# apcamargo/genomad

Measured on NVIDIA H100. Metric: nn_classification_windows_per_s, higher is better.
Workload: dtype split operands on wgmma (conv: fp16 main pass + two e4m3 correction passes; w_v: 3 fp16 passes), fp32 accumulate; fp32-equivalent (<=1e-4 vs the fp32 oracle, measured ~1e-5)

## Files before the change

### genomad_b200/csrc/common.cuh

```cuda
#pragma once
#include <cuda_runtime.h>
#include <cuda_fp16.h>
#include <cuda_fp8.h>
#include <stdint.h>
#include "wgmma.cuh"

namespace gnm {

constexpr int kWindow   = 6000;
constexpr int kTok      = 5997;
constexpr int kVocab    = 257;
constexpr int kC        = 128;
constexpr int kTaps     = 6;
constexpr int kPatches  = 2100;
constexpr int kPatchLen = 4;
constexpr int kPool     = 8;
constexpr int kPooled   = 749;
constexpr int kHidden   = 512;
constexpr float kLeaky  = 0.1f;

constexpr int kRowBytes  = 768;
constexpr int kOffHi16   = 0, kOffLo16 = 256, kOffP8 = 512;
constexpr float kActScale = 32.f;
constexpr float kLo8Scale = 128.f;
constexpr float kHi8Scale = 4.f;
constexpr float kHi8Limit = 448.f / kHi8Scale;
constexpr float kF16Limit = 65504.f;

__device__ __forceinline__ uint32_t smem_u32(const void* p) {
  return static_cast<uint32_t>(__cvta_generic_to_shared(p));
}
__device__ __forceinline__ float lrelu(float x) { return x > 0.f ? x : x * kLeaky; }

__device__ __forceinline__ void split_f16(float x, __half& hi, __half& lo) {
  hi = __float2half_rn(x);
  lo = __float2half_rn(x - __half2float(hi));
}
__device__ __forceinline__ uint32_t pack_h2(__half a, __half b) {
  return static_cast<uint32_t>(__half_as_ushort(a)) | (static_cast<uint32_t>(__half_as_ushort(b)) << 16);
}

__device__ __forceinline__ void split2_f16(float a, float b, __half2& hi, __half2& lo) {
  hi = __floats2half2_rn(a, b);
  const float2 f = __half22float2(hi);
  lo = __floats2half2_rn(a - f.x, b - f.y);
}

__device__ __forceinline__ uint16_t pack_e4m3x2(float a, float b) {
  return static_cast<uint16_t>(__nv_cvt_float2_to_fp8x2(make_float2(a, b), __NV_SATFINITE, __NV_E4M3));
}

__device__ __forceinline__ void stmatrix_x4_trans(uint32_t saddr, uint32_t r0, uint32_t r1, uint32_t r2, uint32_t r3) {
  asm volatile("stmatrix.sync.aligned.m8n8.x4.trans.shared.b16 [%0], {%1, %2, %3, %4};"
               ::"r"(saddr), "r"(r0), "r"(r1), "r"(r2), "r"(r3) : "memory");
}
__device__ __forceinline__ uint4 ld_shared_v4(uint32_t saddr) {
  uint4 v;
  asm volatile("ld.shared.v4.b32 {%0, %1, %2, %3}, [%4];" : "=r"(v.x), "=r"(v.y), "=r"(v.z), "=r"(v.w) : "r"(saddr) : "memory");
  return v;
}

struct DeviceStatus { int code; int info0; int info1; int info2; int act_overflow; int ov_stage[4]; };
enum : int { kDevOk = 0, kDevMbarTimeout = 1 };
__device__ __forceinline__ void flag_act_overflow(DeviceStatus* st, float absmax, float limit, int stage) {
  if (absmax > limit && st) { st->act_overflow = 1; st->ov_stage[stage] = 1; }
}

__device__ __forceinline__ bool elect_one() {
  uint32_t pred;
  asm volatile(
      "{\n\t.reg .pred P;\n\t"
      "elect.sync _|P, 0xffffffff;\n\t"
      "selp.u32 %0, 1, 0, P;\n\t}"
      : "=r"(pred));
  return pred != 0;
}

__device__ __forceinline__ void mbar_init(uint64_t* bar, uint32_t count) {
  asm volatile("mbarrier.init.shared::cta.b64 [%0], %1;" ::"r"(smem_u32(bar)), "r"(count));
}
__device__ __forceinline__ void fence_barrier_init() {
  asm volatile("fence.mbarrier_init.release.cluster;" ::: "memory");
}
__device__ __forceinline__ void fence_proxy_async_smem() {
  asm volatile("fence.proxy.async.shared::cta;" ::: "memory");
}
__device__ __forceinline__ void mbar_arrive_expect_tx(uint64_t* bar, uint32_t bytes) {
  asm volatile("mbarrier.arrive.expect_tx.shared::cta.b64 _, [%0], %1;" ::"r"(smem_u32(bar)), "r"(bytes) : "memory");
}
__device__ __forceinline__ void mbar_arrive(uint64_t* bar) {
  asm volatile("mbarrier.arrive.shared::cta.b64 _, [%0];" ::"r"(smem_u32(bar)) : "memory");
}
__device__ __forceinline__ bool mbar_try_wait(uint64_t* bar, uint32_t parity) {
  uint32_t ok;
  asm volatile(
      "{\n\t.reg .pred p;\n\t"
      "mbarrier.try_wait.parity.shared::cta.b64 p, [%1], %2, %3;\n\t"
      "selp.u32 %0, 1, 0, p;\n\t}"
      : "=r"(ok) : "r"(smem_u32(bar)), "r"(parity), "r"(20000u) : "memory");
  return ok != 0;
}
__device__ __forceinline__ void mbar_wait(uint64_t* bar, uint32_t parity, DeviceStatus* st, int tag) {
  if (mbar_try_wait(bar, parity)) return;
  const long long t0 = clock64();
  for (uint32_t spins = 1;; ++spins) {
    if (mbar_try_wait(bar, parity)) return;
    if ((spins & 255u) == 0 && clock64() - t0 > 4000000000LL) {
      if (st) { st->code = kDevMbarTimeout; st->info0 = tag; st->info1 = blockIdx.x; st->info2 = threadIdx.x; }
      __threadfence_system();
      __trap();
    }
  }
}

__device__ __forceinline__ void tma_prefetch_desc(const void* tmap) {
  asm volatile("prefetch.tensormap [%0];" ::"l"(reinterpret_cast<uint64_t>(tmap)) : "memory");
}
__device__ __forceinline__ uint64_t l2_policy_evict_last() {
  uint64_t p;
  asm volatile("createpolicy.fractional.L2::evict_last.b64 %0, 1.0;" : "=l"(p));
  return p;
}
__device__ __forceinline__ uint64_t l2_policy_evict_first() {
  uint64_t p;
  asm volatile("createpolicy.fractional.L2::evict_first.b64 %0, 1.0;" : "=l"(p));
  return p;
}
__device__ __forceinline__ void tma_load_2d_hint(void* smem_dst, const void* tmap, uint64_t* bar, int c0, int c1, uint64_t policy) {
  asm volatile(
      "cp.async.bulk.tensor.2d.shared::cluster.global.mbarrier::complete_tx::bytes.L2::cache_hint [%0], [%1, {%3, %4}], [%2], %5;"
      ::"r"(smem_u32(smem_dst)), "l"(reinterpret_cast<uint64_t>(tmap)), "r"(smem_u32(bar)), "r"(c0), "r"(c1), "l"(policy)
      : "memory");
}
__device__ __forceinline__ void tma_load_3d_hint(void* smem_dst, const void* tmap, uint64_t* bar, int c0, int c1, int c2, uint64_t policy) {
  asm volatile(
      "cp.async.bulk.tensor.3d.shared::cluster.global.mbarrier::complete_tx::bytes.L2::cache_hint [%0], [%1, {%3, %4, %5}], [%2], %6;"
      ::"r"(smem_u32(smem_dst)), "l"(reinterpret_cast<uint64_t>(tmap)), "r"(smem_u32(bar)), "r"(c0), "r"(c1), "r"(c2), "l"(policy)
      : "memory");
}
}
```

### genomad_b200/csrc/wgmma.cuh

```cuda
#pragma once
#include <stdint.h>

namespace gnm {

__device__ __forceinline__ void wgmma_fence() { asm volatile("wgmma.fence.sync.aligned;" ::: "memory"); }
__device__ __forceinline__ void wgmma_commit() { asm volatile("wgmma.commit_group.sync.aligned;" ::: "memory"); }
template <int kPending> __device__ __forceinline__ void wgmma_wait() {
  asm volatile("wgmma.wait_group.sync.aligned %0;" ::"n"(kPending) : "memory");
}
template <int kN> __device__ __forceinline__ void wgmma_fence_regs(float (&d)[kN]) {
#pragma unroll
  for (int i = 0; i < kN; ++i) asm volatile("" : "+f"(d[i])::"memory");
}

__device__ __forceinline__ uint64_t gmma_desc_sw128(uint32_t saddr) {
  uint64_t d = 0;
  d |= static_cast<uint64_t>((saddr & 0x3FFFF) >> 4);
  d |= static_cast<uint64_t>(1) << 16;
  d |= static_cast<uint64_t>(1024 >> 4) << 32;
  d |= static_cast<uint64_t>(1) << 62;
  return d;
}

#define GNM_ACC8(b) "+f"(d[b]), "+f"(d[b + 1]), "+f"(d[b + 2]), "+f"(d[b + 3]), "+f"(d[b + 4]), "+f"(d[b + 5]), "+f"(d[b + 6]), "+f"(d[b + 7])
__device__ __forceinline__ void wgmma_f16_n48(float (&d)[24], uint64_t da, uint64_t db, uint32_t accumulate) {
  asm volatile("{\n.reg .pred p;\nsetp.ne.b32 p, %26, 0;\n"
               "wgmma.mma_async.sync.aligned.m64n48k16.f32.f16.f16 {%0,%1,%2,%3,%4,%5,%6,%7,%8,%9,%10,%11,%12,%13,%14,%15,%16,%17,%18,%19,%20,%21,%22,%23}, %24,%25,p,1,1,0,0;\n}"
               : GNM_ACC8(0), GNM_ACC8(8), GNM_ACC8(16)
               : "l"(da), "l"(db), "r"(accumulate));
}
__device__ __forceinline__ void wgmma_f16_n192(float (&d)[96], uint64_t da, uint64_t db, uint32_t accumulate) {
  asm volatile("{\n.reg .pred p;\nsetp.ne.b32 p, %98, 0;\n"
               "wgmma.mma_async.sync.aligned.m64n192k16.f32.f16.f16 {%0,%1,%2,%3,%4,%5,%6,%7,%8,%9,%10,%11,%12,%13,%14,%15,%16,%17,%18,%19,%20,%21,%22,%23,%24,%25,%26,%27,%28,%29,%30,%31,%32,%33,%34,%35,%36,%37,%38,%39,%40,%41,%42,%43,%44,%45,%46,%47,%48,%49,%50,%51,%52,%53,%54,%55,%56,%57,%58,%59,%60,%61,%62,%63,%64,%65,%66,%67,%68,%69,%70,%71,%72,%73,%74,%75,%76,%77,%78,%79,%80,%81,%82,%83,%84,%85,%86,%87,%88,%89,%90,%91,%92,%93,%94,%95}, %96,%97,p,1,1,0,0;\n}"
               : GNM_ACC8(0), GNM_ACC8(8), GNM_ACC8(16), GNM_ACC8(24), GNM_ACC8(32), GNM_ACC8(40), GNM_ACC8(48), GNM_ACC8(56), GNM_ACC8(64), GNM_ACC8(72), GNM_ACC8(80), GNM_ACC8(88)
               : "l"(da), "l"(db), "r"(accumulate));
}
__device__ __forceinline__ void wgmma_f16_n256(float (&d)[128], uint64_t da, uint64_t db, uint32_t accumulate) {
  asm volatile("{\n.reg .pred p;\nsetp.ne.b32 p, %130, 0;\n"
               "wgmma.mma_async.sync.aligned.m64n256k16.f32.f16.f16 {%0,%1,%2,%3,%4,%5,%6,%7,%8,%9,%10,%11,%12,%13,%14,%15,%16,%17,%18,%19,%20,%21,%22,%23,%24,%25,%26,%27,%28,%29,%30,%31,%32,%33,%34,%35,%36,%37,%38,%39,%40,%41,%42,%43,%44,%45,%46,%47,%48,%49,%50,%51,%52,%53,%54,%55,%56,%57,%58,%59,%60,%61,%62,%63,%64,%65,%66,%67,%68,%69,%70,%71,%72,%73,%74,%75,%76,%77,%78,%79,%80,%81,%82,%83,%84,%85,%86,%87,%88,%89,%90,%91,%92,%93,%94,%95,%96,%97,%98,%99,%100,%101,%102,%103,%104,%105,%106,%107,%108,%109,%110,%111,%112,%113,%114,%115,%116,%117,%118,%119,%120,%121,%122,%123,%124,%125,%126,%127}, %128,%129,p,1,1,0,0;\n}"
               : GNM_ACC8(0), GNM_ACC8(8), GNM_ACC8(16), GNM_ACC8(24), GNM_ACC8(32), GNM_ACC8(40), GNM_ACC8(48), GNM_ACC8(56), GNM_ACC8(64), GNM_ACC8(72), GNM_ACC8(80), GNM_ACC8(88), GNM_ACC8(96), GNM_ACC8(104), GNM_ACC8(112), GNM_ACC8(120)
               : "l"(da), "l"(db), "r"(accumulate));
}
__device__ __forceinline__ void wgmma_e4m3_n256(float (&d)[128], uint64_t da, uint64_t db, uint32_t accumulate) {
  asm volatile("{\n.reg .pred p;\nsetp.ne.b32 p, %130, 0;\n"
               "wgmma.mma_async.sync.aligned.m64n256k32.f32.e4m3.e4m3 {%0,%1,%2,%3,%4,%5,%6,%7,%8,%9,%10,%11,%12,%13,%14,%15,%16,%17,%18,%19,%20,%21,%22,%23,%24,%25,%26,%27,%28,%29,%30,%31,%32,%33,%34,%35,%36,%37,%38,%39,%40,%41,%42,%43,%44,%45,%46,%47,%48,%49,%50,%51,%52,%53,%54,%55,%56,%57,%58,%59,%60,%61,%62,%63,%64,%65,%66,%67,%68,%69,%70,%71,%72,%73,%74,%75,%76,%77,%78,%79,%80,%81,%82,%83,%84,%85,%86,%87,%88,%89,%90,%91,%92,%93,%94,%95,%96,%97,%98,%99,%100,%101,%102,%103,%104,%105,%106,%107,%108,%109,%110,%111,%112,%113,%114,%115,%116,%117,%118,%119,%120,%121,%122,%123,%124,%125,%126,%127}, %128,%129,p,1,1;\n}"
               : GNM_ACC8(0), GNM_ACC8(8), GNM_ACC8(16), GNM_ACC8(24), GNM_ACC8(32), GNM_ACC8(40), GNM_ACC8(48), GNM_ACC8(56), GNM_ACC8(64), GNM_ACC8(72), GNM_ACC8(80), GNM_ACC8(88), GNM_ACC8(96), GNM_ACC8(104), GNM_ACC8(112), GNM_ACC8(120)
               : "l"(da), "l"(db), "r"(accumulate));
}
__device__ __forceinline__ void wgmma_tf32_n256(float (&d)[128], uint64_t da, uint64_t db, uint32_t accumulate) {
  asm volatile("{\n.reg .pred p;\nsetp.ne.b32 p, %130, 0;\n"
               "wgmma.mma_async.sync.aligned.m64n256k8.f32.tf32.tf32 {%0,%1,%2,%3,%4,%5,%6,%7,%8,%9,%10,%11,%12,%13,%14,%15,%16,%17,%18,%19,%20,%21,%22,%23,%24,%25,%26,%27,%28,%29,%30,%31,%32,%33,%34,%35,%36,%37,%38,%39,%40,%41,%42,%43,%44,%45,%46,%47,%48,%49,%50,%51,%52,%53,%54,%55,%56,%57,%58,%59,%60,%61,%62,%63,%64,%65,%66,%67,%68,%69,%70,%71,%72,%73,%74,%75,%76,%77,%78,%79,%80,%81,%82,%83,%84,%85,%86,%87,%88,%89,%90,%91,%92,%93,%94,%95,%96,%97,%98,%99,%100,%101,%102,%103,%104,%105,%106,%107,%108,%109,%110,%111,%112,%113,%114,%115,%116,%117,%118,%119,%120,%121,%122,%123,%124,%125,%126,%127}, %128,%129,p,1,1;\n}"
               : GNM_ACC8(0), GNM_ACC8(8), GNM_ACC8(16), GNM_ACC8(24), GNM_ACC8(32), GNM_ACC8(40), GNM_ACC8(48), GNM_ACC8(56), GNM_ACC8(64), GNM_ACC8(72), GNM_ACC8(80), GNM_ACC8(88), GNM_ACC8(96), GNM_ACC8(104), GNM_ACC8(112), GNM_ACC8(120)
               : "l"(da), "l"(db), "r"(accumulate));
}
#undef GNM_ACC8

}
```

### genomad_b200/csrc/wv_gather.cuh

```cuda
#pragma once
#include <cuda.h>
#include <type_traits>
#include "common.cuh"
#include "conv_t.cuh"
#include "igloo.cuh"

namespace gnm {

constexpr int kBandRows   = 24;
constexpr int kBandWins   = 8;
constexpr int kWgN        = kBandRows * kBandWins;
constexpr int kNumBands   = (kTok + kBandRows - 1) / kBandRows;
constexpr int kWgRegion   = kWgN * 128;
constexpr int kWgBufs     = 6;
constexpr int kWgSlab     = kWgBufs * kWgRegion;
constexpr int kWgWBytes   = kWvStages * kBStage;
constexpr int kWgMmaWarps = 8;
constexpr int kWgWarps    = 7;
constexpr int kWgThreads  = (kWgMmaWarps + kWgWarps + 1) * 32;
constexpr int kWgGroupCap = 4;
constexpr int kWgGroupMax = 4;
constexpr int kWgSmem     = kWgSlab + kWgWBytes + 2048;
static_assert(kWgSmem <= 232448, "wv_gather_kernel exceeds the 227 KB of shared memory a CTA may use");
static_assert(kWgN == 3 * 64 && kBandRows == 3 * kPool && kBandWins == 8, "unit shape: three pool groups of 8 positions x 8 windows");
static_assert(kWgRegion % 1024 == 0, "regions must keep the 1024-byte alignment of the 128-byte swizzle");

struct WvGatherParams {
  float* q_out;
  float out_scale;
  const int2* grp;
  const int32_t* band_gstart;
  const uint4* wfrag;
  float gather_unscale;
  float* part_t;
  int n_windows, n_pad;
  int groups;
  int n_units;
  const int32_t* cta_split;
  int experiment;
  long long* dbg;
  DeviceStatus* status;
};

__device__ __forceinline__ uint2 ldg_frag(const uint2* p) {
  uint2 v;
  asm volatile("ld.global.nc.L1::evict_last.v2.u32 {%0, %1}, [%2];" : "=r"(v.x), "=r"(v.y) : "l"(p));
  return v;
}
__device__ __forceinline__ void ldsm_x4(uint32_t saddr, uint32_t (&a)[4]) {
  asm volatile("ldmatrix.sync.aligned.m8n8.x4.shared.b16 {%0, %1, %2, %3}, [%4];"
               : "=r"(a[0]), "=r"(a[1]), "=r"(a[2]), "=r"(a[3]) : "r"(saddr));
}
__device__ __forceinline__ void mma_16816(float (&d)[4], const uint32_t (&a)[4], uint32_t b0, uint32_t b1) {
  asm volatile("mma.sync.aligned.m16n8k16.row.col.f32.f16.f16.f32 {%0, %1, %2, %3}, {%4, %5, %6, %7}, {%8, %9}, {%0, %1, %2, %3};"
               : "+f"(d[0]), "+f"(d[1]), "+f"(d[2]), "+f"(d[3]) : "r"(a[0]), "r"(a[1]), "r"(a[2]), "r"(a[3]), "r"(b0), "r"(b1));
}

__global__ void __launch_bounds__(kWgThreads, 1)
wv_gather_kernel(const __grid_constant__ CUtensorMap tm_band, const __grid_constant__ CUtensorMap tm_w, const WvGatherParams p) {
  extern __shared__ uint8_t smem_raw[];
  uint8_t* smem = reinterpret_cast<uint8_t*>((reinterpret_cast<uintptr_t>(smem_raw) + 1023) & ~uintptr_t(1023));
  uint8_t* s_a = smem;
  uint8_t* s_w = smem + kWgSlab;
  uint64_t* bars = reinterpret_cast<uint64_t*>(s_w + kWgWBytes);
  uint64_t* a_full = bars;
  uint64_t* a_empty = bars + 8;
  uint64_t* w_full = bars + 16;

  const int warp = __shfl_sync(0xffffffffu, static_cast<int>(threadIdx.x) >> 5, 0);
  const int lane = threadIdx.x & 31;
  constexpr int kProducerWarp = kWgMmaWarps + kWgWarps;
  const int u_begin = p.cta_split[blockIdx.x], u_end = p.cta_split[blockIdx.x + 1];

  if (warp == kProducerWarp && elect_one()) {
    tma_prefetch_desc(&tm_band);
    tma_prefetch_desc(&tm_w);
    for (int i = 0; i < kWgBufs; ++i) { mbar_init(&a_full[i], 1); mbar_init(&a_empty[i], kWgMmaWarps + kWgWarps); }
    mbar_init(w_full, 1);
    fence_barrier_init();
  }
  __syncthreads();

  if (warp == kProducerWarp) {
    if (elect_one()) {
      mbar_arrive_expect_tx(w_full, kWgWBytes);
      for (int q = 0; q < kWvStages; ++q) tma_load_2d_hint(s_w + q * kBStage, &tm_w, w_full, 0, q * 128, l2_policy_evict_last());
      const uint64_t pol = l2_policy_evict_first();
      uint32_t phases = 0;
      int b0 = 0;
      long long c_wait_empty = 0;
      for (int unit = u_begin; unit < u_end; ++unit) {
        const int band = unit / p.groups;
        const int w0 = (unit - band * p.groups) * kBandWins;
#pragma unroll
        for (int k = 0; k < 4; ++k) {
          int b = b0 + k; if (b >= kWgBufs) b -= kWgBufs;
          const long long tq = clock64();
          mbar_wait(&a_empty[b], ((phases >> b) & 1) ^ 1, p.status, 500 + b);
          c_wait_empty += clock64() - tq;
          phases ^= 1u << b;
          mbar_arrive_expect_tx(&a_full[b], kWgRegion);
          const int src = (k & 1 ? kOffLo16 : kOffHi16) + (k >> 1) * 128;
          tma_load_3d_hint(s_a + b * kWgRegion, &tm_band, &a_full[b], src, w0, band * kBandRows, pol);
        }
        b0 += 4; if (b0 >= kWgBufs) b0 -= kWgBufs;
      }
      if (p.dbg) p.dbg[blockIdx.x * 8 + 7] = c_wait_empty;
    }
  } else if (warp < kWgMmaWarps) {
    const int g = warp >> 2, wq = warp & 3;
    const uint32_t a_base = smem_u32(s_a);
    const uint32_t w_base = smem_u32(s_w) + g * 64 * 128;
    const int ch0 = g * 64 + wq * 16 + (lane >> 2);
    const int win0 = 2 * (lane & 3);
    const float oscale = p.out_scale;
    mbar_wait(w_full, 0, p.status, 510);
    uint32_t phases = 0;
    int b0 = 0;
    uint32_t w_a = 0, t_mma = 0, t_epi = 0;
    float d[96];
    for (int unit = u_begin; unit < u_end; ++unit) {
      auto buf = [&](int k) { const int b = b0 + k; return b >= kWgBufs ? b - kWgBufs : b; };
      const uint32_t t_unit = clock();
#pragma unroll
      for (int kh = 0; kh < 2; ++kh) {
#pragma unroll
        for (int r = 0; r < 2; ++r) {
          const int b = buf(2 * kh + r);
          const uint32_t tq = clock();
          mbar_wait(&a_full[b], (phases >> b) & 1, p.status, 530 + b);
          w_a += clock() - tq;
          phases ^= 1u << b;
        }
        const uint64_t yh = gmma_desc_sw128(a_base + buf(2 * kh) * kWgRegion);
        const uint64_t yl = gmma_desc_sw128(a_base + buf(2 * kh + 1) * kWgRegion);
        const uint64_t whi = gmma_desc_sw128(w_base + (2 * kh) * kBStage);
        const uint64_t wlo = gmma_desc_sw128(w_base + (2 * kh + 1) * kBStage);
        wgmma_fence();
#pragma unroll
        for (int kk = 0; kk < 4; ++kk) {
          wgmma_f16_n192(d, whi + kk * 2, yh + kk * 2, (kh == 0 && kk == 0) ? 0u : 1u);
          wgmma_f16_n192(d, whi + kk * 2, yl + kk * 2, 1u);
        }
#pragma unroll
        for (int kk = 0; kk < 4; ++kk) wgmma_f16_n192(d, wlo + kk * 2, yh + kk * 2, 1u);
        wgmma_commit();
      }
      wgmma_wait<1>();
      __syncwarp();
      if (lane == 0) { mbar_arrive(&a_empty[buf(0)]); mbar_arrive(&a_empty[buf(1)]); }
      wgmma_wait<0>();
      wgmma_fence_regs(d);
      const uint32_t t_epi0 = clock();
      t_mma += t_epi0 - t_unit;
      const int band = unit / p.groups;
      const int w0 = (unit - band * p.groups) * kBandWins;
#pragma unroll
      for (int pg = 0; pg < kBandRows / kPool; ++pg) {
        const int gg = band * (kBandRows / kPool) + pg;
        if (gg < kPooled && !(p.experiment & 128)) {
#pragma unroll
          for (int h = 0; h < 2; ++h)
#pragma unroll
            for (int e = 0; e < 2; ++e) {
              float m = d[32 * pg + 2 * h + e];
#pragma unroll
              for (int i = 1; i < kPool; ++i) m = fmaxf(m, d[32 * pg + 4 * i + 2 * h + e]);
              const int w = w0 + win0 + e;
              if (w < p.n_windows) p.q_out[(static_cast<size_t>(w) * kPooled + gg) * kC + ch0 + 8 * h] = m * oscale;
            }
        }
      }
      __syncwarp();
      if (lane == 0) { mbar_arrive(&a_empty[buf(2)]); mbar_arrive(&a_empty[buf(3)]); }
      t_epi += clock() - t_epi0;
      b0 += 4; if (b0 >= kWgBufs) b0 -= kWgBufs;
    }
    if (p.dbg && warp == 0 && lane == 0) { long long* o = p.dbg + blockIdx.x * 8; o[3] = t_mma; o[4] = w_a; o[6] = t_epi; }
  } else {
    const int gw = warp - kWgMmaWarps;
    const float gscale = p.gather_unscale;
    const int lm_plane = (lane >> 3) & 1, lm_chunk = lane >> 4, lm_win = lane & 7;
    const int gid = lane >> 2, tig = lane & 3;
    const uint32_t slab = smem_u32(s_a);
    int it = 0;
    uint32_t phases = 0;
    int b0 = 0;
    long long c_wait_full = 0, c_gather = 0, tq = 0;
    const long long t_begin = clock64();
    int cur_band = -1, g_first = 0, g_cnt = 0, n_mine = 0;
    int my_e0[kWgGroupCap] = {}, my_meta[kWgGroupCap] = {};
    bool fast = true;
    struct GroupFrag { uint2 b[4]; uint32_t a[4][4]; };
    auto load_group = [&](int e0, int meta, int kh, uint32_t hi_base, uint32_t lo_base, GroupFrag& f) {
      const int row = meta & 31, ne = meta >> 8;
      const uint2* wf = reinterpret_cast<const uint2*>(p.wfrag) + ((static_cast<size_t>(e0 + (gid >> 1)) * 2 + kh) * 16 + tig) * 2 + (gid & 1);
#pragma unroll
      for (int ks = 0; ks < 4; ++ks) f.b[ks] = ((gid >> 1) < ne && !(p.experiment & 1024)) ? ldg_frag(wf + ks * 8) : make_uint2(0u, 0u);
      const uint32_t rb = (lm_plane ? lo_base : hi_base) + row * (kBandWins * 128) + lm_win * 128;
#pragma unroll
      for (int ks = 0; ks < 4; ++ks) {
        if (p.experiment & 2048) { f.a[ks][0] = f.a[ks][1] = f.a[ks][2] = f.a[ks][3] = rb; continue; }
        ldsm_x4(rb + (((ks * 2 + lm_chunk) ^ lm_win) << 4), f.a[ks]);
      }
    };
    auto mma_group = [&](const GroupFrag& f) -> float {
      float d[4][4];
#pragma unroll
      for (int ks = 0; ks < 4; ++ks) d[ks][0] = d[ks][1] = d[ks][2] = d[ks][3] = 0.f;
      if (p.experiment & 256) {
#pragma unroll
        for (int ks = 0; ks < 4; ++ks) asm volatile("" :: "r"(f.a[ks][0] | f.a[ks][1] | f.a[ks][2] | f.a[ks][3] | f.b[ks].x | f.b[ks].y));
      } else {
#pragma unroll
        for (int ks = 0; ks < 4; ++ks) mma_16816(d[ks], f.a[ks], f.b[ks].x, f.b[ks].y);
      }
      float v = 0.f;
#pragma unroll
      for (int ks = 0; ks < 4; ++ks) v += (d[ks][0] + d[ks][2]) + (d[ks][1] + d[ks][3]);
      return v * gscale;
    };
    for (int unit = u_begin; unit < u_end; ++unit, ++it) {
      const int band = unit / p.groups;
      const int w0 = (unit - band * p.groups) * kBandWins;
      if (band != cur_band) {
        cur_band = band;
        g_first = p.band_gstart[band];
        g_cnt = (p.experiment & 32) ? 0 : p.band_gstart[band + 1] - g_first;
        fast = g_cnt <= kWgWarps * kWgGroupCap;
        n_mine = 0;
#pragma unroll
        for (int i = 0; i < kWgGroupCap; ++i) {
          const int gi = gw + i * kWgWarps;
          if (fast && gi < g_cnt) { const int2 m = p.grp[g_first + gi]; my_e0[i] = m.x; my_meta[i] = m.y; n_mine = i + 1; }
        }
      }
      float c0[kWgGroupCap];
#pragma unroll 1
      for (int kh = 0; kh < 2; ++kh) {
        int bh = b0 + 2 * kh; if (bh >= kWgBufs) bh -= kWgBufs;
        int bl = b0 + 2 * kh + 1; if (bl >= kWgBufs) bl -= kWgBufs;
        const uint32_t ph_h = (phases >> bh) & 1, ph_l = (phases >> bl) & 1;
        phases ^= (1u << bh) | (1u << bl);
        const uint32_t hi_base = slab + bh * kWgRegion, lo_base = slab + bl * kWgRegion;
        if (p.dbg) tq = clock64();
        mbar_wait(&a_full[bh], ph_h, p.status, 550 + bh);
        mbar_wait(&a_full[bl], ph_l, p.status, 560 + bl);
        if (p.dbg) { const long long t = clock64(); c_wait_full += t - tq; tq = t; }
        if (fast) {
          auto finish = [&](int i, float v) {
            if (kh == 0) c0[i] = v;
            else if (tig < (my_meta[i] >> 8) && !(p.experiment & 64))
              p.part_t[static_cast<size_t>(my_e0[i] + tig) * p.n_pad + w0 + gid] = c0[i] + v;
          };
#pragma unroll
          for (int i = 0; i < kWgGroupCap; i += 2)
            if (i < n_mine) {
              GroupFrag f0, f1;
              load_group(my_e0[i], my_meta[i], kh, hi_base, lo_base, f0);
              if (i + 1 < n_mine) {
                load_group(my_e0[i + 1], my_meta[i + 1], kh, hi_base, lo_base, f1);
                finish(i, mma_group(f0));
                finish(i + 1, mma_group(f1));
              } else {
                finish(i, mma_group(f0));
              }
            }
        } else {
#pragma unroll 1
          for (int gi = gw; gi < g_cnt; gi += kWgWarps) {
            const int2 m = p.grp[g_first + gi];
            GroupFrag f;
            load_group(m.x, m.y, kh, hi_base, lo_base, f);
            const float v = mma_group(f);
            if (tig < (m.y >> 8)) {
              float* gp = p.part_t + static_cast<size_t>(m.x + tig) * p.n_pad + w0 + gid;
              *gp = kh == 0 ? v : *gp + v;
            }
          }
        }
        __syncwarp();
        if (lane == 0) { mbar_arrive(&a_empty[bh]); mbar_arrive(&a_empty[bl]); }
        if (p.dbg) c_gather += clock64() - tq;
      }
      b0 += 4; if (b0 >= kWgBufs) b0 -= kWgBufs;
    }
    if (p.dbg && warp == kWgMmaWarps && lane == 0) {
      long long* d = p.dbg + blockIdx.x * 8;
      d[0] = clock64() - t_begin; d[1] = c_wait_full; d[2] = c_gather; d[5] = it;
    }
  }
}

__global__ void __launch_bounds__(256)
patch_finish_t_kernel(const float* __restrict__ part_t, const int32_t* __restrict__ slot_of, const float* __restrict__ w_bias,
                      float* __restrict__ mpi, float* __restrict__ mpi_hi, float* __restrict__ mpi_lo, int n_windows, int n_pad) {
  __shared__ float tile[32][33];
  const int p0 = blockIdx.x * 32, w0 = blockIdx.y * 32;
  const int tx = threadIdx.x & 31, ty = threadIdx.x >> 5;
  for (int pp = ty; pp < 32; pp += 8) {
    const int pch = p0 + pp, w = w0 + tx;
    float v = 0.f;
    if (pch < kPatches && w < n_windows) {
      const int4 s4 = *reinterpret_cast<const int4*>(slot_of + pch * 4);
      v = (((part_t[static_cast<size_t>(s4.x) * n_pad + w] + part_t[static_cast<size_t>(s4.y) * n_pad + w]) +
            part_t[static_cast<size_t>(s4.z) * n_pad + w]) + part_t[static_cast<size_t>(s4.w) * n_pad + w]) + w_bias[pch];
    }
    tile[pp][tx] = v;
  }
  __syncthreads();
  for (int ww = ty; ww < 32; ww += 8) {
    const int pch = p0 + tx, w = w0 + ww;
    if (pch < kPatches && w < n_windows) {
      const float v = tile[tx][ww];
      const size_t o = static_cast<size_t>(w) * kPatches + pch;
      mpi[o] = v;
      const float hi = __uint_as_float(__float_as_uint(v) & 0xffffe000u);
      mpi_hi[o] = hi;
      mpi_lo[o] = __uint_as_float(__float_as_uint(v - hi) & 0xffffe000u);
    }
  }
}

}
```

Baseline: 75940.

## Rebalance wv_gather warps with setmaxnreg and split n192 wgmma into two n96

Raises the gather warp count from 7 to 11, so the CTA has 20 warps (640 threads) that split evenly into warpgroups. It uses setmaxnreg to give the MMA warpgroups 128 registers and shrink the producer/gather warpgroups to 72. Each m64n192 wgmma becomes two m64n96 wgmmas over adjacent B columns, and the gather per-warp group cap drops to 3 with one group processed at a time instead of two interleaved. The aim is more gather parallelism to hide the latency of the irregular gather under the fixed register budget. The cost is twice as many wgmma instructions, less instruction-level parallelism per gather warp, and a risk of register spills at 72 registers.

```diff
diff --git a/genomad_b200/csrc/common.cuh b/genomad_b200/csrc/common.cuh
--- a/genomad_b200/csrc/common.cuh
+++ b/genomad_b200/csrc/common.cuh
@@ -76,6 +76,17 @@
   return pred != 0;
 }
 
+template <int kRegs>
+__device__ __forceinline__ void setmaxnreg_inc() {
+  static_assert(kRegs % 8 == 0 && kRegs >= 24 && kRegs <= 256, "setmaxnreg takes a multiple of 8 in [24, 256]");
+  asm volatile("setmaxnreg.inc.sync.aligned.u32 %0;" ::"n"(kRegs));
+}
+template <int kRegs>
+__device__ __forceinline__ void setmaxnreg_dec() {
+  static_assert(kRegs % 8 == 0 && kRegs >= 24 && kRegs <= 256, "setmaxnreg takes a multiple of 8 in [24, 256]");
+  asm volatile("setmaxnreg.dec.sync.aligned.u32 %0;" ::"n"(kRegs));
+}
+
 __device__ __forceinline__ void mbar_init(uint64_t* bar, uint32_t count) {
   asm volatile("mbarrier.init.shared::cta.b64 [%0], %1;" ::"r"(smem_u32(bar)), "r"(count));
 }
diff --git a/genomad_b200/csrc/wgmma.cuh b/genomad_b200/csrc/wgmma.cuh
--- a/genomad_b200/csrc/wgmma.cuh
+++ b/genomad_b200/csrc/wgmma.cuh
@@ -29,10 +29,12 @@
                : GNM_ACC8(0), GNM_ACC8(8), GNM_ACC8(16)
                : "l"(da), "l"(db), "r"(accumulate));
 }
-__device__ __forceinline__ void wgmma_f16_n192(float (&d)[96], uint64_t da, uint64_t db, uint32_t accumulate) {
-  asm volatile("{\n.reg .pred p;\nsetp.ne.b32 p, %98, 0;\n"
-               "wgmma.mma_async.sync.aligned.m64n192k16.f32.f16.f16 {%0,%1,%2,%3,%4,%5,%6,%7,%8,%9,%10,%11,%12,%13,%14,%15,%16,%17,%18,%19,%20,%21,%22,%23,%24,%25,%26,%27,%28,%29,%30,%31,%32,%33,%34,%35,%36,%37,%38,%39,%40,%41,%42,%43,%44,%45,%46,%47,%48,%49,%50,%51,%52,%53,%54,%55,%56,%57,%58,%59,%60,%61,%62,%63,%64,%65,%66,%67,%68,%69,%70,%71,%72,%73,%74,%75,%76,%77,%78,%79,%80,%81,%82,%83,%84,%85,%86,%87,%88,%89,%90,%91,%92,%93,%94,%95}, %96,%97,p,1,1,0,0;\n}"
-               : GNM_ACC8(0), GNM_ACC8(8), GNM_ACC8(16), GNM_ACC8(24), GNM_ACC8(32), GNM_ACC8(40), GNM_ACC8(48), GNM_ACC8(56), GNM_ACC8(64), GNM_ACC8(72), GNM_ACC8(80), GNM_ACC8(88)
+template <int kOff, int kN>
+__device__ __forceinline__ void wgmma_f16_n96(float (&d)[kN], uint64_t da, uint64_t db, uint32_t accumulate) {
+  static_assert(kOff % 8 == 0 && kOff + 48 <= kN, "the 48 accumulator registers must lie inside d");
+  asm volatile("{\n.reg .pred p;\nsetp.ne.b32 p, %50, 0;\n"
+               "wgmma.mma_async.sync.aligned.m64n96k16.f32.f16.f16 {%0,%1,%2,%3,%4,%5,%6,%7,%8,%9,%10,%11,%12,%13,%14,%15,%16,%17,%18,%19,%20,%21,%22,%23,%24,%25,%26,%27,%28,%29,%30,%31,%32,%33,%34,%35,%36,%37,%38,%39,%40,%41,%42,%43,%44,%45,%46,%47}, %48,%49,p,1,1,0,0;\n}"
+               : GNM_ACC8(kOff), GNM_ACC8(kOff + 8), GNM_ACC8(kOff + 16), GNM_ACC8(kOff + 24), GNM_ACC8(kOff + 32), GNM_ACC8(kOff + 40)
                : "l"(da), "l"(db), "r"(accumulate));
 }
 __device__ __forceinline__ void wgmma_f16_n256(float (&d)[128], uint64_t da, uint64_t db, uint32_t accumulate) {
diff --git a/genomad_b200/csrc/wv_gather.cuh b/genomad_b200/csrc/wv_gather.cuh
--- a/genomad_b200/csrc/wv_gather.cuh
+++ b/genomad_b200/csrc/wv_gather.cuh
@@ -16,9 +16,15 @@
 constexpr int kWgSlab     = kWgBufs * kWgRegion;
 constexpr int kWgWBytes   = kWvStages * kBStage;
 constexpr int kWgMmaWarps = 8;
-constexpr int kWgWarps    = 7;
+constexpr int kWgWarps    = 11;
 constexpr int kWgThreads  = (kWgMmaWarps + kWgWarps + 1) * 32;
-constexpr int kWgGroupCap = 4;
+constexpr int kWgRegsLaunch = 65536 / kWgThreads / 8 * 8;
+constexpr int kWgRegsMma    = 128;
+constexpr int kWgRegsGather = 72;
+static_assert(kWgThreads % 128 == 0 && kWgMmaWarps % 4 == 0, "roles must split at warpgroup boundaries: setmaxnreg is per warpgroup");
+static_assert(kWgMmaWarps * 32 * kWgRegsMma + (kWgThreads - kWgMmaWarps * 32) * kWgRegsGather <= kWgThreads * kWgRegsLaunch,
+              "the MMA warpgroups' setmaxnreg.inc would wait forever: the CTA's pool cannot cover it");
+constexpr int kWgGroupCap = 3;
 constexpr int kWgGroupMax = 4;
 constexpr int kWgSmem     = kWgSlab + kWgWBytes + 2048;
 static_assert(kWgSmem <= 232448, "wv_gather_kernel exceeds the 227 KB of shared memory a CTA may use");
@@ -80,34 +86,8 @@
     fence_barrier_init();
   }
   __syncthreads();
-
-  if (warp == kProducerWarp) {
-    if (elect_one()) {
-      mbar_arrive_expect_tx(w_full, kWgWBytes);
-      for (int q = 0; q < kWvStages; ++q) tma_load_2d_hint(s_w + q * kBStage, &tm_w, w_full, 0, q * 128, l2_policy_evict_last());
-      const uint64_t pol = l2_policy_evict_first();
-      uint32_t phases = 0;
-      int b0 = 0;
-      long long c_wait_empty = 0;
-      for (int unit = u_begin; unit < u_end; ++unit) {
-        const int band = unit / p.groups;
-        const int w0 = (unit - band * p.groups) * kBandWins;
-#pragma unroll
-        for (int k = 0; k < 4; ++k) {
-          int b = b0 + k; if (b >= kWgBufs) b -= kWgBufs;
-          const long long tq = clock64();
-          mbar_wait(&a_empty[b], ((phases >> b) & 1) ^ 1, p.status, 500 + b);
-          c_wait_empty += clock64() - tq;
-          phases ^= 1u << b;
-          mbar_arrive_expect_tx(&a_full[b], kWgRegion);
-          const int src = (k & 1 ? kOffLo16 : kOffHi16) + (k >> 1) * 128;
-          tma_load_3d_hint(s_a + b * kWgRegion, &tm_band, &a_full[b], src, w0, band * kBandRows, pol);
-        }
-        b0 += 4; if (b0 >= kWgBufs) b0 -= kWgBufs;
-      }
-      if (p.dbg) p.dbg[blockIdx.x * 8 + 7] = c_wait_empty;
-    }
-  } else if (warp < kWgMmaWarps) {
+  if (warp < kWgMmaWarps) {
+    setmaxnreg_inc<kWgRegsMma>();
     const int g = warp >> 2, wq = warp & 3;
     const uint32_t a_base = smem_u32(s_a);
     const uint32_t w_base = smem_u32(s_w) + g * 64 * 128;
@@ -122,6 +102,10 @@
     for (int unit = u_begin; unit < u_end; ++unit) {
       auto buf = [&](int k) { const int b = b0 + k; return b >= kWgBufs ? b - kWgBufs : b; };
       const uint32_t t_unit = clock();
+      auto mma = [&](uint64_t da, uint64_t db, uint32_t acc) {
+        wgmma_f16_n96<0>(d, da, db, acc);
+        wgmma_f16_n96<48>(d, da, db + ((96 * 128) >> 4), acc);
+      };
 #pragma unroll
       for (int kh = 0; kh < 2; ++kh) {
 #pragma unroll
@@ -139,11 +123,11 @@
         wgmma_fence();
 #pragma unroll
         for (int kk = 0; kk < 4; ++kk) {
-          wgmma_f16_n192(d, whi + kk * 2, yh + kk * 2, (kh == 0 && kk == 0) ? 0u : 1u);
-          wgmma_f16_n192(d, whi + kk * 2, yl + kk * 2, 1u);
-        }
-#pragma unroll
-        for (int kk = 0; kk < 4; ++kk) wgmma_f16_n192(d, wlo + kk * 2, yh + kk * 2, 1u);
+          mma(whi + kk * 2, yh + kk * 2, (kh == 0 && kk == 0) ? 0u : 1u);
+          mma(whi + kk * 2, yl + kk * 2, 1u);
+        }
+#pragma unroll
+        for (int kk = 0; kk < 4; ++kk) mma(wlo + kk * 2, yh + kk * 2, 1u);
         wgmma_commit();
       }
       wgmma_wait<1>();
@@ -178,116 +162,139 @@
     }
     if (p.dbg && warp == 0 && lane == 0) { long long* o = p.dbg + blockIdx.x * 8; o[3] = t_mma; o[4] = w_a; o[6] = t_epi; }
   } else {
-    const int gw = warp - kWgMmaWarps;
-    const float gscale = p.gather_unscale;
-    const int lm_plane = (lane >> 3) & 1, lm_chunk = lane >> 4, lm_win = lane & 7;
-    const int gid = lane >> 2, tig = lane & 3;
-    const uint32_t slab = smem_u32(s_a);
-    int it = 0;
-    uint32_t phases = 0;
-    int b0 = 0;
-    long long c_wait_full = 0, c_gather = 0, tq = 0;
-    const long long t_begin = clock64();
-    int cur_band = -1, g_first = 0, g_cnt = 0, n_mine = 0;
-    int my_e0[kWgGroupCap] = {}, my_meta[kWgGroupCap] = {};
-    bool fast = true;
-    struct GroupFrag { uint2 b[4]; uint32_t a[4][4]; };
-    auto load_group = [&](int e0, int meta, int kh, uint32_t hi_base, uint32_t lo_base, GroupFrag& f) {
-      const int row = meta & 31, ne = meta >> 8;
-      const uint2* wf = reinterpret_cast<const uint2*>(p.wfrag) + ((static_cast<size_t>(e0 + (gid >> 1)) * 2 + kh) * 16 + tig) * 2 + (gid & 1);
-#pragma unroll
-      for (int ks = 0; ks < 4; ++ks) f.b[ks] = ((gid >> 1) < ne && !(p.experiment & 1024)) ? ldg_frag(wf + ks * 8) : make_uint2(0u, 0u);
-      const uint32_t rb = (lm_plane ? lo_base : hi_base) + row * (kBandWins * 128) + lm_win * 128;
-#pragma unroll
-      for (int ks = 0; ks < 4; ++ks) {
-        if (p.experiment & 2048) { f.a[ks][0] = f.a[ks][1] = f.a[ks][2] = f.a[ks][3] = rb; continue; }
-        ldsm_x4(rb + (((ks * 2 + lm_chunk) ^ lm_win) << 4), f.a[ks]);
-      }
-    };
-    auto mma_group = [&](const GroupFrag& f) -> float {
-      float d[4][4];
-#pragma unroll
-      for (int ks = 0; ks < 4; ++ks) d[ks][0] = d[ks][1] = d[ks][2] = d[ks][3] = 0.f;
-      if (p.experiment & 256) {
-#pragma unroll
-        for (int ks = 0; ks < 4; ++ks) asm volatile("" :: "r"(f.a[ks][0] | f.a[ks][1] | f.a[ks][2] | f.a[ks][3] | f.b[ks].x | f.b[ks].y));
-      } else {
-#pragma unroll
-        for (int ks = 0; ks < 4; ++ks) mma_16816(d[ks], f.a[ks], f.b[ks].x, f.b[ks].y);
-      }
-      float v = 0.f;
-#pragma unroll
-      for (int ks = 0; ks < 4; ++ks) v += (d[ks][0] + d[ks][2]) + (d[ks][1] + d[ks][3]);
-      return v * gscale;
-    };
-    for (int unit = u_begin; unit < u_end; ++unit, ++it) {
-      const int band = unit / p.groups;
-      const int w0 = (unit - band * p.groups) * kBandWins;
-      if (band != cur_band) {
-        cur_band = band;
-        g_first = p.band_gstart[band];
-        g_cnt = (p.experiment & 32) ? 0 : p.band_gstart[band + 1] - g_first;
-        fast = g_cnt <= kWgWarps * kWgGroupCap;
-        n_mine = 0;
-#pragma unroll
-        for (int i = 0; i < kWgGroupCap; ++i) {
-          const int gi = gw + i * kWgWarps;
-          if (fast && gi < g_cnt) { const int2 m = p.grp[g_first + gi]; my_e0[i] = m.x; my_meta[i] = m.y; n_mine = i + 1; }
-        }
-      }
-      float c0[kWgGroupCap];
+    setmaxnreg_dec<kWgRegsGather>();
+    if (warp == kProducerWarp) {
+      if (elect_one()) {
+        mbar_arrive_expect_tx(w_full, kWgWBytes);
+        for (int q = 0; q < kWvStages; ++q) tma_load_2d_hint(s_w + q * kBStage, &tm_w, w_full, 0, q * 128, l2_policy_evict_last());
+        const uint64_t pol = l2_policy_evict_first();
+        uint32_t phases = 0;
+        int b0 = 0;
+        long long c_wait_empty = 0;
+        for (int unit = u_begin; unit < u_end; ++unit) {
+          const int band = unit / p.groups;
+          const int w0 = (unit - band * p.groups) * kBandWins;
+#pragma unroll
+          for (int k = 0; k < 4; ++k) {
+            int b = b0 + k; if (b >= kWgBufs) b -= kWgBufs;
+            const long long tq = clock64();
+            mbar_wait(&a_empty[b], ((phases >> b) & 1) ^ 1, p.status, 500 + b);
+            c_wait_empty += clock64() - tq;
+            phases ^= 1u << b;
+            mbar_arrive_expect_tx(&a_full[b], kWgRegion);
+            const int src = (k & 1 ? kOffLo16 : kOffHi16) + (k >> 1) * 128;
+            tma_load_3d_hint(s_a + b * kWgRegion, &tm_band, &a_full[b], src, w0, band * kBandRows, pol);
+          }
+          b0 += 4; if (b0 >= kWgBufs) b0 -= kWgBufs;
+        }
+        if (p.dbg) p.dbg[blockIdx.x * 8 + 7] = c_wait_empty;
+      }
+    } else {
+      const int gw = warp - kWgMmaWarps;
+      const float gscale = p.gather_unscale;
+      const int lm_plane = (lane >> 3) & 1, lm_chunk = lane >> 4, lm_win = lane & 7;
+      const int gid = lane >> 2, tig = lane & 3;
+      const uint32_t slab = smem_u32(s_a);
+      int it = 0;
+      uint32_t phases = 0;
+      int b0 = 0;
+      long long c_wait_full = 0, c_gather = 0, tq = 0;
+      const long long t_begin = clock64();
+      int cur_band = -1, g_first = 0, g_cnt = 0, n_mine = 0;
+      int my_e0[kWgGroupCap] = {}, my_meta[kWgGroupCap] = {};
+      bool fast = true;
+      struct GroupFrag { uint2 b[4]; uint32_t a[4][4]; };
+      auto load_group = [&](int e0, int meta, int kh, uint32_t hi_base, uint32_t lo_base, GroupFrag& f) {
+        const int row = meta & 31, ne = meta >> 8;
+        const uint2* wf = reinterpret_cast<const uint2*>(p.wfrag) + ((static_cast<size_t>(e0 + (gid >> 1)) * 2 + kh) * 16 + tig) * 2 + (gid & 1);
+#pragma unroll
+        for (int ks = 0; ks < 4; ++ks) f.b[ks] = ((gid >> 1) < ne && !(p.experiment & 1024)) ? ldg_frag(wf + ks * 8) : make_uint2(0u, 0u);
+        const uint32_t rb = (lm_plane ? lo_base : hi_base) + row * (kBandWins * 128) + lm_win * 128;
+#pragma unroll
+        for (int ks = 0; ks < 4; ++ks) {
+          if (p.experiment & 2048) { f.a[ks][0] = f.a[ks][1] = f.a[ks][2] = f.a[ks][3] = rb; continue; }
+          ldsm_x4(rb + (((ks * 2 + lm_chunk) ^ lm_win) << 4), f.a[ks]);
+        }
+      };
+      auto mma_group = [&](const GroupFrag& f) -> float {
+        float d[4][4];
+#pragma unroll
+        for (int ks = 0; ks < 4; ++ks) d[ks][0] = d[ks][1] = d[ks][2] = d[ks][3] = 0.f;
+        if (p.experiment & 256) {
+#pragma unroll
+          for (int ks = 0; ks < 4; ++ks) asm volatile("" :: "r"(f.a[ks][0] | f.a[ks][1] | f.a[ks][2] | f.a[ks][3] | f.b[ks].x | f.b[ks].y));
+        } else {
+#pragma unroll
+          for (int ks = 0; ks < 4; ++ks) mma_16816(d[ks], f.a[ks], f.b[ks].x, f.b[ks].y);
+        }
+        float v = 0.f;
+#pragma unroll
+        for (int ks = 0; ks < 4; ++ks) v += (d[ks][0] + d[ks][2]) + (d[ks][1] + d[ks][3]);
+        return v * gscale;
+      };
+      for (int unit = u_begin; unit < u_end; ++unit, ++it) {
+        const int band = unit / p.groups;
+        const int w0 = (unit - band * p.groups) * kBandWins;
+        if (band != cur_band) {
+          cur_band = band;
+          g_first = p.band_gstart[band];
+          g_cnt = (p.experiment & 32) ? 0 : p.band_gstart[band + 1] - g_first;
+          fast = g_cnt <= kWgWarps * kWgGroupCap;
+          n_mine = 0;
+#pragma unroll
+          for (int i = 0; i < kWgGroupCap; ++i) {
+            const int gi = gw + i * kWgWarps;
+            if (fast && gi < g_cnt) { const int2 m = p.grp[g_first + gi]; my_e0[i] = m.x; my_meta[i] = m.y; n_mine = i + 1; }
+          }
+        }
+        float c0[kWgGroupCap];
 #pragma unroll 1
-      for (int kh = 0; kh < 2; ++kh) {
-        int bh = b0 + 2 * kh; if (bh >= kWgBufs) bh -= kWgBufs;
-        int bl = b0 + 2 * kh + 1; if (bl >= kWgBufs) bl -= kWgBufs;
-        const uint32_t ph_h = (phases >> bh) & 1, ph_l = (phases >> bl) & 1;
-        phases ^= (1u << bh) | (1u << bl);
-        const uint32_t hi_base = slab + bh * kWgRegion, lo_base = slab + bl * kWgRegion;
-        if (p.dbg) tq = clock64();
-        mbar_wait(&a_full[bh], ph_h, p.status, 550 + bh);
-        mbar_wait(&a_full[bl], ph_l, p.status, 560 + bl);
-        if (p.dbg) { const long long t = clock64(); c_wait_full += t - tq; tq = t; }
-        if (fast) {
-          auto finish = [&](int i, float v) {
-            if (kh == 0) c0[i] = v;
-            else if (tig < (my_meta[i] >> 8) && !(p.experiment & 64))
-              p.part_t[static_cast<size_t>(my_e0[i] + tig) * p.n_pad + w0 + gid] = c0[i] + v;
-          };
-#pragma unroll
-          for (int i = 0; i < kWgGroupCap; i += 2)
-            if (i < n_mine) {
-              GroupFrag f0, f1;
-              load_group(my_e0[i], my_meta[i], kh, hi_base, lo_base, f0);
-              if (i + 1 < n_mine) {
-                load_group(my_e0[i + 1], my_meta[i + 1], kh, hi_base, lo_base, f1);
-                finish(i, mma_group(f0));
-                finish(i + 1, mma_group(f1));
-              } else {
-                finish(i, mma_group(f0));
+        for (int kh = 0; kh < 2; ++kh) {
+          int bh = b0 + 2 * kh; if (bh >= kWgBufs) bh -= kWgBufs;
+          int bl = b0 + 2 * kh + 1; if (bl >= kWgBufs) bl -= kWgBufs;
+          const uint32_t ph_h = (phases >> bh) & 1, ph_l = (phases >> bl) & 1;
+          phases ^= (1u << bh) | (1u << bl);
+          const uint32_t hi_base = slab + bh * kWgRegion, lo_base = slab + bl * kWgRegion;
+          if (p.dbg) tq = clock64();
+          mbar_wait(&a_full[bh], ph_h, p.status, 550 + bh);
+          mbar_wait(&a_full[bl], ph_l, p.status, 560 + bl);
+          if (p.dbg) { const long long t = clock64(); c_wait_full += t - tq; tq = t; }
+          if (fast) {
+            auto finish = [&](int i, float v) {
+              if (kh == 0) c0[i] = v;
+              else if (tig < (my_meta[i] >> 8) && !(p.experiment & 64))
+                p.part_t[static_cast<size_t>(my_e0[i] + tig) * p.n_pad + w0 + gid] = c0[i] + v;
+            };
+#pragma unroll
+            for (int i = 0; i < kWgGroupCap; ++i)
+              if (i < n_mine) {
+                GroupFrag f;
+                load_group(my_e0[i], my_meta[i], kh, hi_base, lo_base, f);
+                finish(i, mma_group(f));
+              }
+          } else {
+#pragma unroll 1
+            for (int gi = gw; gi < g_cnt; gi += kWgWarps) {
+              const int2 m = p.grp[g_first + gi];
+              GroupFrag f;
+              load_group(m.x, m.y, kh, hi_base, lo_base, f);
+              const float v = mma_group(f);
+              if (tig < (m.y >> 8)) {
+                float* gp = p.part_t + static_cast<size_t>(m.x + tig) * p.n_pad + w0 + gid;
+                *gp = kh == 0 ? v : *gp + v;
               }
             }
-        } else {
-#pragma unroll 1
-          for (int gi = gw; gi < g_cnt; gi += kWgWarps) {
-            const int2 m = p.grp[g_first + gi];
-            GroupFrag f;
-            load_group(m.x, m.y, kh, hi_base, lo_base, f);
-            const float v = mma_group(f);
-            if (tig < (m.y >> 8)) {
-              float* gp = p.part_t + static_cast<size_t>(m.x + tig) * p.n_pad + w0 + gid;
-              *gp = kh == 0 ? v : *gp + v;
-            }
           }
-        }
-        __syncwarp();
-        if (lane == 0) { mbar_arrive(&a_empty[bh]); mbar_arrive(&a_empty[bl]); }
-        if (p.dbg) c_gather += clock64() - tq;
-      }
-      b0 += 4; if (b0 >= kWgBufs) b0 -= kWgBufs;
-    }
-    if (p.dbg && warp == kWgMmaWarps && lane == 0) {
-      long long* d = p.dbg + blockIdx.x * 8;
-      d[0] = clock64() - t_begin; d[1] = c_wait_full; d[2] = c_gather; d[5] = it;
+          __syncwarp();
+          if (lane == 0) { mbar_arrive(&a_empty[bh]); mbar_arrive(&a_empty[bl]); }
+          if (p.dbg) c_gather += clock64() - tq;
+        }
+        b0 += 4; if (b0 >= kWgBufs) b0 -= kWgBufs;
+      }
+      if (p.dbg && warp == kWgMmaWarps && lane == 0) {
+        long long* d = p.dbg + blockIdx.x * 8;
+        d[0] = clock64() - t_begin; d[1] = c_wait_full; d[2] = c_gather; d[5] = it;
+      }
     }
   }
 }
```

New measurement: 75550, median of 6. About the same (-0.5%).
